# Shibodd/volume_path_tracer

Measured on AMD Instinct MI355X. Metric: Msamples/s (whole node) + achieved HBM GB/s, wdas_cloud 1920×1080, higher is better.
Workload: dtype f32

## Files before the change

### __graft_entry__.py

```python
from __future__ import annotations

import subprocess
import sys
from pathlib import Path

ROOT = Path(__file__).resolve().parent


def build() -> None:
    sys.path.insert(0, str(ROOT))
    from volume_path_tracer_amd import build as B

    B.build(verbose=True)
    subprocess.run(["make", "-s", "-C", str(ROOT / "oracle")], check=True)
    subprocess.run(["make", "-s", "-C", str(ROOT / "tests" / "native")], check=True)
    subprocess.run([sys.executable, "-B", "-c", "import sys; sys.path[:0] = [%r, %r]; import alpha_lib, denoise_lib; "
                    "alpha_lib.build_lib(); denoise_lib.build_lib()" % (str(ROOT), str(ROOT / "tests"))], check=True)
    import volume_path_tracer_amd
    from volume_path_tracer_amd import capi

    capi.lib()


def smoke() -> None:
    sys.path.insert(0, str(ROOT))
    sys.path.insert(0, str(ROOT / "tests"))
    import numpy as np
    import torch

    import oracle_lib as O
    from volume_path_tracer_amd.render import Integrator
    from volume_path_tracer_amd.scenes import SynthGrid, workload

    assert torch.cuda.is_available(), "smoke() needs a HIP device"
    wl = workload("c4", width=32, height=24, spp=2, grid_n=64)
    dens, temp = SynthGrid(1, 64).grid(), SynthGrid(2, 64).grid()
    it = Integrator(wl.cfg, dens, temp, device=0)
    jobs = wl.cfg.jobs_per_wave() * 2
    rec = torch.full((jobs * 64, 3), float("nan"), device="cuda:0")
    it.render_jobs(0, jobs, records=rec)
# ... 15 lines not shown
```

### include/vpt_gpu.h

```cpp
#ifndef VPT_GPU_H
#define VPT_GPU_H

#include <stddef.h>
#include <stdint.h>

#ifdef __cplusplus
extern "C" {
#endif

#define VPT_ABI_VERSION 1

enum {
  VPT_OK = 0,
  VPT_E_INVALID = 1,
  VPT_E_HIP = 2,
  VPT_E_IO = 3,
  VPT_E_PARSE = 4,
  VPT_E_NOMEM = 5,
  VPT_E_STATE = 6
};


typedef struct vpt_camera_params {
  float position[3];
// ... 98 lines not shown
int vpt_gpu_create(const vpt_configuration* cfg, const vpt_grid_desc* density,
                   const vpt_grid_desc* temperature, const float* blackbody_500x3, int device,
                   vpt_gpu_ctx** out);
int vpt_gpu_create_many(const vpt_configuration* cfg, const vpt_grid_desc* density,
                        const vpt_grid_desc* temperature, const float* blackbody_500x3, const int* devices, int n,
                        vpt_gpu_ctx** out);
typedef struct vpt_host_grids vpt_host_grids;
int vpt_grids_flatten(const vpt_grid_desc* density, const vpt_grid_desc* temperature, vpt_host_grids** out);
int vpt_gpu_create_from(const vpt_configuration* cfg, const vpt_host_grids* grids, const float* blackbody_500x3,
                        const int* devices, int n, vpt_gpu_ctx** out);
void vpt_grids_free(vpt_host_grids* grids);
int vpt_gpu_destroy(vpt_gpu_ctx* ctx);

int vpt_gpu_job_space(const vpt_gpu_ctx* ctx, uint64_t* jobs_per_wave, uint64_t* total_jobs);

int vpt_gpu_render_jobs(vpt_gpu_ctx* ctx, uint64_t jid_begin, uint64_t jid_count,
                        float* film_device, void* hip_stream);

enum { VPT_FILM_ATOMIC = 0, VPT_FILM_ORDERED = 1 };
int vpt_gpu_set_film_order(vpt_gpu_ctx* ctx, int mode, uint64_t max_bytes);
int vpt_gpu_film_order_info(const vpt_gpu_ctx* ctx, int* mode, uint64_t* buffer_bytes, uint64_t* ordered_launches,
                            uint64_t* atomic_launches);

int vpt_gpu_render_tiles(vpt_gpu_ctx* ctx, uint32_t tile_lo, uint32_t tile_hi, uint64_t wave_begin,
                         uint64_t wave_count, float* film_device, void* hip_stream);

int vpt_gpu_set_film_moments(vpt_gpu_ctx* ctx, float* m2_device);

int vpt_gpu_render_tile_list(vpt_gpu_ctx* ctx, const uint32_t* tiles, uint32_t n, uint64_t wave_begin,
                             uint64_t wave_count, float* film_device, void* hip_stream);

int vpt_gpu_tile_errors(vpt_gpu_ctx* ctx, const float* film_device, const float* m2_device, float abs_floor,
                        float* err_T_host, void* hip_stream);

typedef struct vpt_adaptive_params {
  float target_error, abs_floor;
  uint32_t min_waves, step_waves, max_waves;
} vpt_adaptive_params;

typedef struct vpt_adaptive_result {
  uint32_t rounds, tiles_at_max;
  uint64_t jobs_rendered, jobs_uniform;
  float max_error;
} vpt_adaptive_result;

int vpt_gpu_render_adaptive(vpt_gpu_ctx* ctx, const vpt_adaptive_params* p, float* film_device, float* m2_device,
// ... 138 lines not shown
```

### volume_path_tracer_amd/capi.py

```python
from __future__ import annotations

import ctypes as C
import os
from pathlib import Path

import numpy as np

PKG_DIR = Path(__file__).resolve().parent
LIB_DIR = PKG_DIR / "lib"
LIB_PATH = Path(os.environ["VPT_LIB"]) if os.environ.get("VPT_LIB") else LIB_DIR / "libvpt_amd.so"

VPT_OK = 0
VPT_BLACKBODY_ROWS = 500


class CameraParams(C.Structure):
    _fields_ = [("position", C.c_float * 3), ("look", C.c_float * 3), ("up", C.c_float * 3),
                ("vfov_deg", C.c_float), ("imaging_ratio", C.c_float)]


class WorkerParams(C.Structure):
    _fields_ = [("single_pixel_enabled", C.c_int32), ("use_jitter", C.c_int32),
                ("single_pixel_coord", C.c_int64 * 2),
                ("infinite_light_xyz", C.c_float * 3), ("infinite_light_multiplier", C.c_float),
# ... 75 lines not shown
    def make(cls, iterations=4, n_guides=0, sigma_l=4.0, rel_floor=1e-3, guide_sigma=None):
        if guide_sigma is None:
            guide_sigma = 0.2
        if np.isscalar(guide_sigma):
            guide_sigma = [guide_sigma] * n_guides
        gs = [float(v) for v in guide_sigma][:4]
        if len(gs) < min(n_guides, 4):
            raise ValueError("denoise: one guide_sigma per guide")
        gs += [1.0] * (4 - len(gs))
        return cls(int(iterations), int(n_guides), float(sigma_l), float(rel_floor), (C.c_float * 4)(*gs))


assert C.sizeof(DenoiseParams) == 32

EVENT_DTYPE = np.dtype([("jid", "<u8"), ("pixel", "<u4"), ("seq", "<u4"), ("type", "<u4"), ("v", "<f4", (7,))])
assert EVENT_DTYPE.itemsize == 48
DDA_ROW_DTYPE = np.dtype([("ijk", "<i4", (3,)), ("t", "<f4"), ("value", "<f4"), ("dim_getdim", "<u4"),
                          ("dim_nodeinfo", "<u4"), ("active", "<i4"), ("maximum", "<f4")])
assert DDA_ROW_DTYPE.itemsize == 36
VPT_RNG_REFERENCE, VPT_RNG_PIXEL = 0, 1
VPT_ORDER_JID, VPT_ORDER_COST_WAVE_MAJOR, VPT_ORDER_COST_TILE_MAJOR, VPT_ORDER_COST_TAIL = 0, 1, 2, 3
VPT_ORDER_COST_SAME_TILE = 4
VPT_FILM_ATOMIC, VPT_FILM_ORDERED = 0, 1
VPT_GATES_CONTEXT, VPT_GATES_LATENCY, VPT_GATES_FULL = 0, 1, 2
EVENT_NAMES = ("new_ray", "sampled_point", "null", "scatter_terminated", "scatter", "absorbed")


def _ptr(arr, ctype):
    if arr is None:
        return C.cast(None, C.POINTER(ctype))
    return arr.ctypes.data_as(C.POINTER(ctype))


class Grid:

    def __init__(self, *, map_mat, map_inv_mat, map_vec, background, bbox_min, bbox_max,
                 leaf_origin, leaf_values, leaf_max, leaf_value_mask=None,
                 tile_origin=None, tile_level=None, tile_value=None, tile_active=None,
                 lower_origin=None, upper_origin=None):
        self.leaf_origin = np.ascontiguousarray(leaf_origin, dtype=np.int32).reshape(-1, 3)
        n = self.leaf_origin.shape[0]
        self.leaf_values = np.ascontiguousarray(leaf_values, dtype=np.float32).reshape(n, 512)
        self.leaf_max = np.ascontiguousarray(leaf_max, dtype=np.float32).reshape(n)
        if leaf_value_mask is None:
            leaf_value_mask = np.full((n, 8), np.uint64(0xFFFFFFFFFFFFFFFF), dtype=np.uint64)
        self.leaf_value_mask = np.ascontiguousarray(leaf_value_mask, dtype=np.uint64).reshape(n, 8)
# ... 130 lines not shown
    if hasattr(L, "vpt_gpu_gate_info"):
        L.vpt_gpu_gate_info.argtypes = [vp, C.c_int, C.POINTER(C.c_int), C.POINTER(C.c_int)]
    L.vpt_gpu_launch_info.argtypes = [vp, C.POINTER(C.c_int), C.POINTER(C.c_int)]
    L.vpt_last_error.restype = C.c_char_p
    L.vpt_synth_grid.argtypes = [C.c_int, C.c_int]
    L.vpt_synth_grid.restype = gridp
    L.vpt_synth_free.argtypes = [gridp]
    L.vpt_grid_from_nanovdb.argtypes = [C.c_void_p, C.c_size_t, C.POINTER(gridp)]
    L.vpt_grid_read_nvdb.argtypes = [C.c_char_p, C.c_char_p, C.POINTER(gridp)]
    L.vpt_grid_free.argtypes = [gridp]
    L.vpt_film_to_srgb8.argtypes = [fp, C.c_int64, C.c_int64, C.POINTER(C.c_uint8)]
    L.vpt_gpu_trace_jobs.argtypes = [vp, C.c_uint64, C.c_uint64, vp, vp, C.c_uint64, C.POINTER(C.c_uint64), vp]
    L.vpt_gpu_majorant_trace.argtypes = [vp, fp, fp, fp, C.c_int, C.POINTER(C.c_int)]
    L.vpt_dda_trace.argtypes = [C.POINTER(GridDesc), fp, fp, vp, C.c_int, C.POINTER(C.c_int)]
    L.vpt_gpu_set_rng_mode.argtypes = [vp, C.c_int]
    if hasattr(L, "vpt_gpu_set_pixel_chunk"):
        L.vpt_gpu_set_pixel_chunk.argtypes = [vp, C.c_int]
    L.vpt_gpu_set_run_skipping.argtypes = [vp, C.c_int]
    L.vpt_gpu_kernel_variant.argtypes = [vp, C.POINTER(C.c_int), C.POINTER(C.c_int)]
    if hasattr(L, "vpt_gpu_set_film_order"):
        L.vpt_gpu_set_film_order.argtypes = [vp, C.c_int, C.c_uint64]
        L.vpt_gpu_film_order_info.argtypes = [vp, C.POINTER(C.c_int), C.POINTER(C.c_uint64),
                                              C.POINTER(C.c_uint64), C.POINTER(C.c_uint64)]
    L.vpt_gpu_set_job_order.argtypes = [vp, C.c_int]
    L.vpt_gpu_set_job_order_tail.argtypes = [vp, C.c_int]
    L.vpt_gpu_tile_costs.argtypes = [vp, fp, C.POINTER(C.c_uint32)]
    L.vpt_gpu_set_tile_costs.argtypes = [vp, fp]
    L.vpt_gpu_set_job_permutation.argtypes = [vp, C.POINTER(C.c_uint32), C.c_uint64]
    if hasattr(L, "vpt_gpu_set_latency_kernel"):
        L.vpt_gpu_set_latency_kernel.argtypes = [vp, C.c_int, C.c_int]
    if hasattr(L, "vpt_gpu_set_compaction"):
        L.vpt_gpu_set_compaction.argtypes = [vp, C.c_int]
        L.vpt_gpu_latency_kernel_info.argtypes = [vp, C.POINTER(C.c_int), C.POINTER(C.c_int)]
    if hasattr(L, "vpt_gpu_bind_thread_near"):
        L.vpt_gpu_bind_thread_near.argtypes = [vp, C.POINTER(C.c_int)]
    if hasattr(L, "vpt_gpu_stream_create"):
        L.vpt_gpu_stream_create.argtypes = [vp, C.POINTER(vp)]
        L.vpt_gpu_stream_destroy.argtypes = [vp, vp]
        L.vpt_gpu_stream_sync.argtypes = [vp, vp]
        L.vpt_gpu_film_alloc.argtypes = [vp, C.POINTER(vp)]
        L.vpt_gpu_film_free.argtypes = [vp, vp]
        L.vpt_gpu_film_flush_to_host.argtypes = [vp, vp, fp]
    if hasattr(L, "vpt_gpu_feed_open"):
        L.vpt_gpu_feed_open.argtypes = [vp, vp, vp, C.c_uint64, C.POINTER(vp)]
        L.vpt_gpu_feed_push.argtypes = [vp, C.POINTER(C.c_uint64), C.c_uint64]
        L.vpt_gpu_feed_close.argtypes = [vp]
# ... 45 lines not shown
```

### volume_path_tracer_amd/csrc/vpt_ctx.h

```cpp
#pragma once

#include <hip/hip_runtime.h>

#include <atomic>
#include <chrono>
#include <cstdint>
#include <mutex>
#include <string>
#include <vector>

#include "vpt_internal.h"
#include "vpt_launch.h"

#define VPT_HIP(call)                                                                                 \
  do {                                                                                                \
    hipError_t e_ = (call);                                                                           \
    if (e_ != hipSuccess)                                                                             \
      return ::vpt::set_error(VPT_E_HIP, std::string(#call " failed: ") + hipGetErrorString(e_));            \
  } while (0)

#ifndef VPT_DEFAULT_JOB_ORDER
#define VPT_DEFAULT_JOB_ORDER VPT_ORDER_COST_SAME_TILE
#endif

#ifndef VPT_DEFAULT_FULL_GATE_IDLE
#define VPT_DEFAULT_FULL_GATE_IDLE 4
#endif

#ifndef VPT_RUNS_MIN_FRACTION
#define VPT_RUNS_MIN_FRACTION 0.25
#endif

namespace vpt {
struct DeviceGrid {
  void* cells8 = nullptr;
  void* runs8 = nullptr;
  void* walk8 = nullptr;
  double run_fraction = 0.0;
  void* cells128 = nullptr;
  void* root = nullptr;
  void* bricks = nullptr;
  DevGrid dev{};
  size_t bytes = 0;
};

}

namespace vpt {
struct FeedLaunch {
  const uint64_t* word;
  uint64_t* ring;
  uint64_t mask;
  unsigned* error;
  uint64_t* started;
  uint64_t* waiting;
  uint32_t* tile_done;
};
struct BandLaunch {
  uint32_t tile_lo, tiles, waves, group;
  bool list = false;
};
}

struct vpt_gpu_feed;

struct vpt_gpu_ctx {
// ... 48 lines not shown
  hipEvent_t samples_done = nullptr;
  bool samples_used = false;
  uint64_t ordered_launches = 0, atomic_launches = 0;
  uint32_t* band_rank = nullptr;
  uint32_t band_rank_lo = 0, band_rank_hi = 0;
  uint32_t* list_dev = nullptr;
  uint32_t* list_slot_dev = nullptr;
  std::vector<uint32_t> list_host, list_slot_host;
  bool list_ranked = false;
  float* m2 = nullptr;
  float* tile_err = nullptr;
  float* gang_scratch = nullptr;
  uint64_t gang_scratch_bytes = 0;
  uint32_t* gang_waves = nullptr;
  void* denoise_scratch = nullptr;
  uint64_t denoise_scratch_bytes = 0;
  hipEvent_t denoise_done = nullptr;
  bool denoise_used = false;
  std::mutex denoise_mu;
  uint64_t frame_waves = 0, frame_jid_lo = 0;
  uint32_t frame_tile_lo = 0, frame_tiles = 0;
  float* frame_film = nullptr;
  double setup_ms[5] = {};
};

struct vpt_gpu_feed {
  vpt_gpu_ctx* ctx = nullptr;
  hipStream_t stream = nullptr;
  float* film = nullptr;
  uint64_t* block = nullptr;
  uint64_t* word = nullptr;
  uint32_t* error = nullptr;
  uint64_t* started = nullptr;
  uint64_t* waiting = nullptr;
  uint64_t* ring = nullptr;
  uint32_t* counts = nullptr;
  bool stage = false;
  uint32_t* done_dev = nullptr;
  float* pin_film = nullptr;
  uint32_t* pin_done = nullptr;
  std::vector<float> shown;
  std::vector<uint32_t> shown_done;
  hipStream_t copy_stream = nullptr;
  hipStream_t own_stream = nullptr;
  bool ring_clean = false;
  uint64_t cap = 0;
// ... 22 lines not shown
```

### volume_path_tracer_amd/csrc/vpt_gpu.hip

```cpp
#include <hip/hip_runtime.h>
#include <pthread.h>
#include <sched.h>
#include <unistd.h>

#include <algorithm>
#include <cmath>
#include <cstdio>
#include <cstdlib>
#include <cstring>
#include <fstream>
#include <functional>
#include <memory>
#include <atomic>
#include <mutex>
#include <chrono>
#include <string>
#include <thread>
#include <vector>

#include "vpt_ctx.h"
#include "vpt_kernels.h"
#include "vpt_denoise.h"

namespace vpt {
// ... 25 lines not shown
  int rc;
  const size_t need = h.cells8.size() * sizeof(int2) + h.runs8.size() + h.walk8.size() * sizeof(uint32_t) +
                      h.cells128.size() * sizeof(int2) + h.root.size() * sizeof(RootTileDev) +
                      h.bricks.size() * sizeof(float);
  size_t free_b = 0, total_b = 0;
  VPT_HIP(hipMemGetInfo(&free_b, &total_b));
  if (need > free_b)
    return set_error(VPT_E_NOMEM, "grid upload: needs " + std::to_string(need >> 20) + " MiB (" +
                                      std::to_string(h.dev.leaf_count) + " leaves x 9 KiB stencil pool + tables), " +
                                      std::to_string(free_b >> 20) + " MiB free on the device");
  if ((rc = upload(h.cells8.data(), h.cells8.size() * sizeof(int2), &d.cells8, d.bytes))) return rc;
  if ((rc = upload(h.runs8.data(), h.runs8.size(), &d.runs8, d.bytes))) return rc;
  if ((rc = upload(h.walk8.data(), h.walk8.size() * sizeof(uint32_t), &d.walk8, d.bytes))) return rc;
  d.run_fraction = h.run_fraction;
  if ((rc = upload(h.cells128.data(), h.cells128.size() * sizeof(int2), &d.cells128, d.bytes))) return rc;
  if ((rc = upload(h.root.data(), h.root.size() * sizeof(RootTileDev), &d.root, d.bytes))) return rc;
  if ((rc = upload(h.bricks.data(), h.bricks.size() * sizeof(float), &d.bricks, d.bytes))) return rc;
  d.dev.cells8 = (const int2*)d.cells8;
  d.dev.runs8 = (const uint8_t*)d.runs8;
  d.dev.walk8 = (const uint32_t*)d.walk8;
  d.dev.cells128 = (const int2*)d.cells128;
  d.dev.root = (const RootTileDev*)d.root;
  d.dev.bricks = (const float*)d.bricks;
  return VPT_OK;
}

static void free_grid(DeviceGrid& d) {
  (void)hipFree(d.cells8);
  (void)hipFree(d.runs8);
  (void)hipFree(d.walk8);
  (void)hipFree(d.cells128);
  (void)hipFree(d.root);
  (void)hipFree(d.bricks);
  d = DeviceGrid{};
}

}

namespace {

constexpr int kProfWords = 2 * vpt::PB_COUNT + vpt::PT_COUNT;
constexpr uint32_t kLaunchSlots = 64;
constexpr uint64_t kSpreadLanes = 6;

int wait_ctx(vpt_gpu_ctx* ctx);

int push_scene(vpt_gpu_ctx* ctx) {
  int rc = wait_ctx(ctx);
  if (rc) return rc;
  vpt::DevScene lat = ctx->scene;
  lat.gate_min = ctx->lat_gate[0];
  lat.gate_idle = ctx->lat_gate[1];
  lat.gate_eval = ctx->lat_gate[2];
  lat.gate_walk = ctx->lat_gate[3];
  lat.wave_lanes = ctx->lat_wave_lanes;
  VPT_HIP(hipMemcpyAsync(ctx->scene_dev, &ctx->scene, sizeof(vpt::DevScene), hipMemcpyHostToDevice, ctx->stream));
  VPT_HIP(hipMemcpyAsync(ctx->scene_lat_dev, &lat, sizeof(vpt::DevScene), hipMemcpyHostToDevice, ctx->stream));
// ... 133 lines not shown
  if (ctx->samples) {
    (void)hipFree(ctx->samples);
    ctx->samples = nullptr;
    ctx->samples_bytes = 0;
  }
  const hipError_t e = hipMalloc((void**)&ctx->samples, bytes);
  if (e != hipSuccess) {
    ctx->samples = nullptr;
    (void)hipGetLastError();
    return vpt::set_error(VPT_E_NOMEM, "ordered film: " + std::to_string(bytes >> 20) + " MiB sample buffer: " +
                                           hipGetErrorString(e) + " (vpt_gpu_set_film_order's max_bytes splits launches)");
  }
  ctx->samples_bytes = bytes;
  out = ctx->samples;
  return VPT_OK;
}

uint64_t ordered_cap(vpt_gpu_ctx* ctx, uint64_t want) {
  if (ctx->film_order_max) return ctx->film_order_max;
  if (want <= ctx->samples_bytes) return ctx->samples_bytes;
  size_t free_b = 0, total_b = 0;
  if (hipMemGetInfo(&free_b, &total_b) != hipSuccess) return ctx->samples_bytes;
  return (uint64_t)(free_b + ctx->samples_bytes) / 4 * 3;
}

}

int vpt::host::ctx_device(vpt_gpu_ctx* ctx) {
  hipError_t e = hipSetDevice(ctx->device);
  if (e != hipSuccess) return vpt::set_error(VPT_E_HIP, std::string("hipSetDevice: ") + hipGetErrorString(e));
  return VPT_OK;
}

int vpt::host::launch_tile_counts(vpt_gpu_ctx* ctx, float* film, const uint32_t* counts_dev, hipStream_t s) {
  const uint64_t npix = (uint64_t)ctx->scene.W * (uint64_t)ctx->scene.H;
  hipLaunchKernelGGL(vpt::vpt_tile_count_kernel, dim3((unsigned)((npix + 255) / 256)), dim3(256), 0, s, ctx->scene_dev,
                     film, counts_dev);
  VPT_HIP(hipGetLastError());
  return VPT_OK;
}

int vpt::host::render(vpt_gpu_ctx* ctx, uint64_t jid_begin, uint64_t jid_count, float* film, float* records,
                      void* stream_ptr, vpt_event* events, uint64_t event_cap, uint32_t* slot_out,
                      const vpt::FeedLaunch* feed, const vpt::BandLaunch* band) {
  if (!ctx) return vpt::set_error(VPT_E_INVALID, "render: null context");
  int rc = ctx_device(ctx);
// ... 332 lines not shown
  ctx->device = device;
  ctx->cfg = *cfg;
  ctx->setup_ms[0] = grids.flatten_ms;
  using clk = std::chrono::steady_clock;
  auto t = clk::now();
  auto lap = [&](int i) {
    const auto now = clk::now();
    ctx->setup_ms[i] += std::chrono::duration<double, std::milli>(now - t).count();
    t = now;
  };
  int rc = ctx_device(ctx.get());
  if (rc) return rc;
  lap(4);
  if ((rc = vpt::build_scene(*cfg, ctx->scene))) return rc;
  if ((rc = vpt::upload_grid(grids.density, ctx->density))) return rc;
  if (grids.has_temperature && (rc = vpt::upload_grid(grids.temperature, ctx->temperature))) return rc;
  lap(1);
  const bool has_temperature = grids.has_temperature;
  ctx->use_runs = !has_temperature && ctx->density.run_fraction >= VPT_RUNS_MIN_FRACTION;
  ctx->scene.density = ctx->density.dev;
  vpt::scene_finalize(ctx->scene);
  ctx->scene.temperature = ctx->temperature.dev;
  ctx->scene.has_temperature = has_temperature ? 1 : 0;
  ctx->scene.bb_lds_ok = has_temperature ? vpt::blackbody_rows_suffice(grids.temp_range, cfg->volume_parameters.temperature_scale,
                                                                    cfg->volume_parameters.temperature_offset, vpt::kBbLdsRows)
                                     : 0;

  std::vector<float> bb(501 * 3, 0.0f);
  if (blackbody_500x3)
    std::memcpy(bb.data(), blackbody_500x3, 500 * 3 * sizeof(float));
  else
    vpt::blackbody_table(bb.data());
  size_t scratch = 0;
  if ((rc = vpt::upload(bb.data(), bb.size() * sizeof(float), (void**)&ctx->bb, scratch))) return rc;
  if ((rc = vpt::upload(vpt::cie_table(), 471 * 3 * sizeof(float), (void**)&ctx->cie, scratch))) return rc;
  ctx->scene.bb = ctx->bb;
  ctx->scene.cie = ctx->cie;

  ctx->film_count = (uint64_t)cfg->output_size[0] * (uint64_t)cfg->output_size[1] * 4;
  VPT_HIP(hipMalloc((void**)&ctx->film, ctx->film_count * sizeof(float)));
  VPT_HIP(hipMemset(ctx->film, 0, ctx->film_count * sizeof(float)));
  VPT_HIP(hipMalloc((void**)&ctx->job_counter, kLaunchSlots * 2 * sizeof(unsigned long long)));
  for (uint32_t i = 0; i < kLaunchSlots; ++i)
    VPT_HIP(hipEventCreateWithFlags(&ctx->slot_done[i], hipEventDisableTiming));
  VPT_HIP(hipMalloc((void**)&ctx->counters, vpt::kCounterCount * sizeof(unsigned long long)));
  VPT_HIP(hipMemset(ctx->counters, 0, vpt::kCounterCount * sizeof(unsigned long long)));
// ... 594 lines not shown

int vpt_gpu_set_pixel_chunk(vpt_gpu_ctx* ctx, int chunk) {
  if (!ctx || chunk < 0 || (chunk & (chunk - 1)) != 0 || (chunk > 0 && ctx->scene.tile_area % (uint32_t)chunk != 0))
    return vpt::set_error(VPT_E_INVALID, "vpt_gpu_set_pixel_chunk: 0 or a power of two dividing the tile area");
  ctx->pixel_chunk = chunk;
  return VPT_OK;
}

int vpt_gpu_set_run_skipping(vpt_gpu_ctx* ctx, int mode) {
  if (!ctx || mode < -1 || mode > 1) return vpt::set_error(VPT_E_INVALID, "vpt_gpu_set_run_skipping: bad argument");
  if (mode == 1 && ctx->scene.has_temperature)
    return vpt::set_error(VPT_E_INVALID, "vpt_gpu_set_run_skipping: no run-skipping variant with a temperature grid");
  ctx->use_runs = mode < 0 ? (!ctx->scene.has_temperature && ctx->density.run_fraction >= VPT_RUNS_MIN_FRACTION) : mode == 1;
  return VPT_OK;
}

int vpt_gpu_kernel_variant(const vpt_gpu_ctx* ctx, int* has_temperature, int* run_skipping) {
  if (!ctx) return vpt::set_error(VPT_E_INVALID, "null context");
  if (has_temperature) *has_temperature = ctx->scene.has_temperature ? 1 : 0;
  if (run_skipping) *run_skipping = ctx->use_runs ? 1 : 0;
  return VPT_OK;
}

int vpt_gpu_set_film_order(vpt_gpu_ctx* ctx, int mode, uint64_t max_bytes) {
  if (!ctx || (mode != VPT_FILM_ATOMIC && mode != VPT_FILM_ORDERED))
    return vpt::set_error(VPT_E_INVALID, "vpt_gpu_set_film_order: bad argument");
  int rc = ctx_device(ctx);
  if (rc) return rc;
  ctx->film_order = mode;
  ctx->film_order_max = max_bytes;
  if (mode == VPT_FILM_ATOMIC && ctx->samples && ctx->open_feeds.load() == 0) {
    if (ctx->samples_used) VPT_HIP(hipEventSynchronize(ctx->samples_done));
    (void)hipFree(ctx->samples);
    ctx->samples = nullptr;
    ctx->samples_bytes = 0;
  }
  return VPT_OK;
}

int vpt_gpu_film_order_info(const vpt_gpu_ctx* ctx, int* mode, uint64_t* buffer_bytes, uint64_t* ordered_launches,
                            uint64_t* atomic_launches) {
  if (!ctx) return vpt::set_error(VPT_E_INVALID, "null context");
  if (mode) *mode = ctx->film_order;
  if (buffer_bytes) *buffer_bytes = ctx->samples_bytes;
  if (ordered_launches) *ordered_launches = ctx->ordered_launches;
  if (atomic_launches) *atomic_launches = ctx->atomic_launches;
// ... 403 lines not shown
```

### volume_path_tracer_amd/csrc/vpt_integrator.h

```cpp
#pragma once

#include <hip/hip_runtime.h>
#include <stdint.h>

#include "vpt_math.h"

namespace vpt {

struct RootTileDev {
  int32_t origin[3];
  float value;
  int32_t active;
  int32_t pad[3];
};

struct DevGrid {
  float mat[9], inv_mat[9], vec[3];
  float background;
  int32_t bbox_min[3], bbox_max[3];
  int32_t r8_org[3], r8_n[3];
  int32_t w8_org[3], w8_n[3];
  uint32_t w8_max;
  int32_t r128_org[3], r128_n[3];
  int32_t root_count, leaf_count;
  const int2* cells8;
  const uint8_t* runs8;
  const uint32_t* walk8;
  const int2* cells128;
  const RootTileDev* root;
  const float* bricks;
};

constexpr int kBrickVox = 576 * 4;
__host__ __device__ __forceinline__ int64_t brick_index(int32_t code, int32_t i, int32_t j, int32_t k) {
  return ((int64_t)code * 576 + ((j & 7) * 8 + (k & 7)) * 9 + (i & 7)) * 4;
}

struct Cell {
  int32_t code;
  float value;
};

__host__ __device__ __forceinline__ int32_t local_const(int32_t c) {
#if defined(__HIP_DEVICE_COMPILE__)
  int32_t r;
  asm volatile("v_mov_b32 %0, %1" : "=v"(r) : "i"(c));
  return r;
#else
  return c;
#endif
}
__host__ __device__ __forceinline__ float local_const(float c) {
#if defined(__HIP_DEVICE_COMPILE__)
  return __builtin_bit_cast(float, local_const(__builtin_bit_cast(int32_t, c)));
#else
  return c;
#endif
}
// ... 84 lines not shown
    v[1] = lo.y;
    v[2] = lo.z;
    v[3] = lo.w;
    v[4] = hi.x;
    v[5] = hi.y;
    v[6] = hi.z;
    v[7] = hi.w;
  } else {
#pragma unroll 1
    for (int q = 0; q < 8; ++q) {
      const float val = value_at(g, i + (q >> 2), j + ((q >> 1) & 1), k + (q & 1));
      v[0] = q == 0 ? val : v[0];
      v[1] = q == 1 ? val : v[1];
      v[2] = q == 2 ? val : v[2];
      v[3] = q == 3 ? val : v[3];
      v[4] = q == 4 ? val : v[4];
      v[5] = q == 5 ? val : v[5];
      v[6] = q == 6 ? val : v[6];
      v[7] = q == 7 ? val : v[7];
    }
  }
}

__host__ __device__ __forceinline__ float lerpf(float a, float b, float w) { return a + w * (b - a); }
__host__ __device__ __forceinline__ bool trilinear(const DevGrid& g, StencilCell& last, float x, float y, float z,
                                                   float& out) {
  float fi = floorf(x), fj = floorf(y), fk = floorf(z);
  float u = x - fi, v = y - fj, w = z - fk;
  int32_t i = (int32_t)fi, j = (int32_t)fj, k = (int32_t)fk;
  bool refresh = i != last.i || j != last.j || k != last.k;
  const int32_t dx = (i ^ last.i) | (j ^ last.j) | (k ^ last.k);
  const bool same_leaf = last.code >= 0 && dx >= 0 && dx < 8;
  Cell c;
  if (same_leaf) {
    c.code = last.code;
    c.value = 0.0f;
  } else {
    c = cell_at(g, i, j, k);
  }
  last.i = i;
  last.j = j;
  last.k = k;
  last.code = c.code;
  float s[8];
  fetch_stencil(g, c, i, j, k, s);
  out = lerpf(lerpf(lerpf(s[0], s[1], w), lerpf(s[2], s[3], w), v), lerpf(lerpf(s[4], s[5], w), lerpf(s[6], s[7], w), v), u);
  return refresh;
}
constexpr int32_t kNoCell = (int32_t)0x80000000;

__host__ __device__ __forceinline__ void map_inv(const DevGrid& g, float x, float y, float z, float& ox, float& oy, float& oz) {
  const float* m = g.inv_mat;
  float a = x - g.vec[0], b = y - g.vec[1], c = z - g.vec[2];
// ... 551 lines not shown
  if (u < 0.0f) {
    u = rng_uniform(ln.rng);
    if (Debug) env.tally(CNT_RNG_DRAWS, 1);
  }
  float total = ((0.0f + p_n) + p_a) + p_s;
  float uu = u * total;
  int ev;
  uu -= p_n;
  if (uu <= 0) {
    ev = 0;
  } else {
    uu -= p_a;
    ev = (uu <= 0) ? 1 : 2;
  }
  if (ev == 1) {
    if (Debug) env.event(ln, VPT_EV_ABSORBED, nullptr, nullptr, 0.0f);
    ln.state = ST_FINISH_T;
  } else if (ev == 2) {
    if (lc.depth++ >= S.max_depth) {
      if (Debug) env.event(ln, VPT_EV_SCATTER_TERMINATED, nullptr, nullptr, 0.0f);
      ln.state = ST_FINISH_T;
    } else {
      if (Debug) env.tally(CNT_SCATTERS, 1);
      for (int i = 0; i < 3; ++i) lc.ro[i] = cp[i];
      if (S.li_zero) {
        lc.Tr = -1.0f;
        ln.state = ST_NEE_DONE;
      } else {
        lc.Tr = local_const(1.0f);
        ln.shadow = 1;
        ln.state = ST_SHADOW;
      }
    }
  }
  if (Debug && ev == 0) env.event(ln, VPT_EV_NULL, nullptr, nullptr, 0.0f);
  if (ev != 0) ln.sm = SM_NONE;
}

template <bool HasTemp, bool Debug, class Env>
__host__ __device__ __forceinline__ void eval_collision(ScenePtr sp, const DevScene& S, const DevGrid& G, Lane& ln, Env& env) {
  LaneCold& lc = env.cold();
  const float sigma_maj = ln.s_dmaj * S.sigma_t;
  {
    const float dt_m = -math::logf_glibc_unit(lc.y_draw, env.logf_table()) / sigma_maj;
    const float tc = ln.s_t0 + math::div_by_recip(dt_m, ln.scale, ln.rscale);
    if (!(tc < ln.s_t1)) {
// ... 480 lines not shown
```

### volume_path_tracer_amd/csrc/vpt_kernels.h

```cpp
#pragma once

#include <hip/hip_runtime.h>

#include "vpt_alpha.h"
#include "vpt_internal.h"
#include "vpt_launch.h"

namespace vpt {

constexpr int kCounterCount = CNT_COUNT;
#ifndef VPT_WAVES_FAST
#define VPT_WAVES_FAST 7
#endif
#ifndef VPT_WAVES_SLOW
#define VPT_WAVES_SLOW 4
#endif
#ifndef VPT_WAVES_TEMP
#define VPT_WAVES_TEMP 6
#endif
#ifndef VPT_WAVES_LAT
#define VPT_WAVES_LAT 4
#endif

__shared__ LaneCold g_lane_cold[kBlockThreads];
// ... 984 lines not shown
    for (int i = 0; i < 3; ++i) dv[i] = S.cam_t[i] + (S.cam_L[i * 3] * rx + S.cam_L[i * 3 + 1] * ry);
    const float n = sqrtf(dv[0] * dv[0] + dv[1] * dv[1] + dv[2] * dv[2]);
    if (!(n > 0.0f)) continue;
    for (int i = 0; i < 3; ++i) dv[i] /= n;
    Lane ln;
    lane_init(ln);
    if (!begin_ray(G, ln, S.cam_pos, ray_dir_setup(G, dv))) continue;
    int steps = 0;
    float tau = 0.0f;
    while (ln.s_t1 < ln.T1 && steps < (1 << 16)) {
      begin_segment(ln);
      bool done;
      do {
        ++steps;
        done = hdda_step(G, ln);
      } while (!done && steps < (1 << 16));
      tau += S.sigma_t * ln.s_dmaj * (ln.s_t1 - ln.s_t0) * ln.scale;
    }
    c += (float)steps + 4.0f * tau;
  }
  cost[tile] = c;
}

__global__ __launch_bounds__(64) void vpt_alpha_kernel(const DevScene* scene, const uint32_t* rank, uint32_t sub,
                                                       float* alpha, float* tau) {
  const DevScene& S = *scene;
  const uint32_t area = S.tile_area, chunks = (area + 63u) / 64u;
  const uint32_t tb = blockIdx.x / chunks, q = (blockIdx.x - tb * chunks) * 64u + threadIdx.x;
  if ((uint64_t)tb >= S.T) return;
  const uint32_t t = rank[tb];
  const int32_t x0 = (int32_t)(t % (uint32_t)S.ntx) * S.tw, y0 = (int32_t)(t / (uint32_t)S.ntx) * S.th;
  const int32_t rw = min(S.W - x0, S.tw), rh = min(S.H - y0, S.th);
  if (q >= area || (int32_t)q >= rw * rh) return;
  const int32_t yl = (int32_t)q / rw, px = x0 + ((int32_t)q - yl * rw), py = y0 + yl;
  if (S.single_pixel_enabled && (px != S.sp_x || py != S.sp_y)) return;
  float a, od;
  alpha_pixel(S, px, py, sub, a, od);
  const uint64_t p = (uint64_t)py * (uint64_t)S.W + (uint64_t)px;
  alpha[p] = a;
  if (tau) tau[p] = od;
}

}
```

### volume_path_tracer_amd/render.py

```python
from __future__ import annotations

import ctypes as C
import threading
import time
from typing import Optional

import numpy as np

from . import capi


def ceildiv(a: int, b: int) -> int:
    return a // b + (a % b != 0)


class TileProvider:

    def __init__(self, img_size, waves: int, tile_size):
        self.img_w, self.img_h = int(img_size[0]), int(img_size[1])
        self.tile_w, self.tile_h = int(tile_size[0]), int(tile_size[1])
        self.ntx, self.nty = ceildiv(self.img_w, self.tile_w), ceildiv(self.img_h, self.tile_h)
        self.num_tiles = self.ntx * self.nty
        self.requested_waves = int(waves)
        self.max_wave_idx = 0
# ... 273 lines not shown

    def set_compaction(self, every: int) -> None:
        capi.check(capi.lib().vpt_gpu_set_compaction(self.h, int(every)), "vpt_gpu_set_compaction")

    def latency_kernel_info(self) -> dict:
        m, b = C.c_int(), C.c_int()
        capi.check(capi.lib().vpt_gpu_latency_kernel_info(self.h, C.byref(m), C.byref(b)), "vpt_gpu_latency_kernel_info")
        return {"mode": int(m.value), "resident_blocks_per_cu": int(b.value)}

    def kernel_variant(self) -> dict:
        t, r = C.c_int(), C.c_int()
        capi.check(capi.lib().vpt_gpu_kernel_variant(self.h, C.byref(t), C.byref(r)), "vpt_gpu_kernel_variant")
        return {"has_temperature": bool(t.value), "run_skipping": bool(r.value)}

    def set_film_order(self, mode: int, max_bytes: int = 0) -> None:
        capi.check(capi.lib().vpt_gpu_set_film_order(self.h, int(mode), int(max_bytes)), "vpt_gpu_set_film_order")

    def film_order_info(self) -> dict:
        m, b, o, a = C.c_int(), C.c_uint64(), C.c_uint64(), C.c_uint64()
        capi.check(capi.lib().vpt_gpu_film_order_info(self.h, C.byref(m), C.byref(b), C.byref(o), C.byref(a)),
                   "vpt_gpu_film_order_info")
        return {"mode": int(m.value), "buffer_bytes": int(b.value), "ordered_launches": int(o.value),
                "atomic_launches": int(a.value)}

    def set_job_order(self, mode: int) -> None:
        capi.check(capi.lib().vpt_gpu_set_job_order(self.h, int(mode)), "vpt_gpu_set_job_order")

    def set_job_order_tail(self, waves: int) -> None:
        capi.check(capi.lib().vpt_gpu_set_job_order_tail(self.h, int(waves)), "vpt_gpu_set_job_order_tail")

    def tile_costs(self):
        T = self.cfg.jobs_per_wave()
        cost, rank = np.zeros(T, np.float32), np.zeros(T, np.uint32)
        capi.check(capi.lib().vpt_gpu_tile_costs(self.h, cost.ctypes.data_as(C.POINTER(C.c_float)),
                                                  rank.ctypes.data_as(C.POINTER(C.c_uint32))), "vpt_gpu_tile_costs")
        return cost, rank

    def set_tile_costs(self, cost) -> None:
        c = np.ascontiguousarray(cost, np.float32)
        assert c.shape == (self.cfg.jobs_per_wave(),)
        capi.check(capi.lib().vpt_gpu_set_tile_costs(self.h, c.ctypes.data_as(C.POINTER(C.c_float))),
                   "vpt_gpu_set_tile_costs")

    def set_job_permutation(self, perm) -> None:
        p = np.ascontiguousarray(perm if perm is not None else [], np.uint32)
        capi.check(capi.lib().vpt_gpu_set_job_permutation(self.h, p.ctypes.data_as(C.POINTER(C.c_uint32)), p.size),
# ... 172 lines not shown
```

Baseline: 1675.

## Add dense stencil brick pool to bypass sparse cell lookup in trilinear sampling

Adds an optional dense pool holding a full 8^3 stencil brick for every cell of the level-8 grid, filled at setup by an expand kernel that copies the sparse bricks and synthesises the stencils for empty cells. Trilinear lookups inside the dense bounds then read two float4 directly from this pool and skip the cell/leaf indirection. An AUTO policy turns it on when the pool fits within one eighth of device memory. This trades extra memory and a one-time expansion pass for fewer dependent loads per sample. It also re-maps the scatter position through the density transform when temperature is present.

After: 1714 (median of 6 runs). 1.02x the previous value.

```diff
diff --git a/__graft_entry__.py b/__graft_entry__.py
--- a/__graft_entry__.py
+++ b/__graft_entry__.py
@@ -14,8 +14,9 @@
     B.build(verbose=True)
     subprocess.run(["make", "-s", "-C", str(ROOT / "oracle")], check=True)
     subprocess.run(["make", "-s", "-C", str(ROOT / "tests" / "native")], check=True)
-    subprocess.run([sys.executable, "-B", "-c", "import sys; sys.path[:0] = [%r, %r]; import alpha_lib, denoise_lib; "
-                    "alpha_lib.build_lib(); denoise_lib.build_lib()" % (str(ROOT), str(ROOT / "tests"))], check=True)
+    subprocess.run([sys.executable, "-B", "-c", "import sys; sys.path[:0] = [%r, %r]; import alpha_lib, denoise_lib, "
+                    "dense_pool_lib; alpha_lib.build_lib(); denoise_lib.build_lib(); dense_pool_lib.build_program()"
+                    % (str(ROOT), str(ROOT / "tests"))], check=True)
     import volume_path_tracer_amd
     from volume_path_tracer_amd import capi
 
diff --git a/include/vpt_gpu.h b/include/vpt_gpu.h
--- a/include/vpt_gpu.h
+++ b/include/vpt_gpu.h
@@ -144,6 +144,13 @@
 int vpt_gpu_film_order_info(const vpt_gpu_ctx* ctx, int* mode, uint64_t* buffer_bytes, uint64_t* ordered_launches,
                             uint64_t* atomic_launches);
 
+enum { VPT_POOL_SPARSE = 0, VPT_POOL_DENSE = 1, VPT_POOL_AUTO = 2 };
+int vpt_gpu_set_pool_layout(vpt_gpu_ctx* ctx, int layout);
+int vpt_gpu_set_pool_cap(vpt_gpu_ctx* ctx, uint64_t max_bytes);
+int vpt_gpu_pool_info(const vpt_gpu_ctx* ctx, int* layout, int* policy, uint64_t* sparse_bytes, uint64_t* dense_bytes,
+                      double* expand_ms);
+int vpt_gpu_debug_read_pool(vpt_gpu_ctx* ctx, int grid, uint64_t cell_begin, uint64_t cell_count, float* out);
+
 int vpt_gpu_render_tiles(vpt_gpu_ctx* ctx, uint32_t tile_lo, uint32_t tile_hi, uint64_t wave_begin,
                          uint64_t wave_count, float* film_device, void* hip_stream);
 
diff --git a/volume_path_tracer_amd/capi.py b/volume_path_tracer_amd/capi.py
--- a/volume_path_tracer_amd/capi.py
+++ b/volume_path_tracer_amd/capi.py
@@ -121,6 +121,7 @@
 VPT_ORDER_JID, VPT_ORDER_COST_WAVE_MAJOR, VPT_ORDER_COST_TILE_MAJOR, VPT_ORDER_COST_TAIL = 0, 1, 2, 3
 VPT_ORDER_COST_SAME_TILE = 4
 VPT_FILM_ATOMIC, VPT_FILM_ORDERED = 0, 1
+VPT_POOL_SPARSE, VPT_POOL_DENSE, VPT_POOL_AUTO = 0, 1, 2
 VPT_GATES_CONTEXT, VPT_GATES_LATENCY, VPT_GATES_FULL = 0, 1, 2
 EVENT_NAMES = ("new_ray", "sampled_point", "null", "scatter_terminated", "scatter", "absorbed")
 
@@ -297,6 +298,12 @@
         L.vpt_gpu_set_film_order.argtypes = [vp, C.c_int, C.c_uint64]
         L.vpt_gpu_film_order_info.argtypes = [vp, C.POINTER(C.c_int), C.POINTER(C.c_uint64),
                                               C.POINTER(C.c_uint64), C.POINTER(C.c_uint64)]
+    if hasattr(L, "vpt_gpu_set_pool_layout"):
+        L.vpt_gpu_set_pool_layout.argtypes = [vp, C.c_int]
+        L.vpt_gpu_set_pool_cap.argtypes = [vp, C.c_uint64]
+        L.vpt_gpu_pool_info.argtypes = [vp, C.POINTER(C.c_int), C.POINTER(C.c_int), C.POINTER(C.c_uint64),
+                                        C.POINTER(C.c_uint64), C.POINTER(C.c_double)]
+        L.vpt_gpu_debug_read_pool.argtypes = [vp, C.c_int, C.c_uint64, C.c_uint64, fp]
     L.vpt_gpu_set_job_order.argtypes = [vp, C.c_int]
     L.vpt_gpu_set_job_order_tail.argtypes = [vp, C.c_int]
     L.vpt_gpu_tile_costs.argtypes = [vp, fp, C.POINTER(C.c_uint32)]
diff --git a/volume_path_tracer_amd/csrc/vpt_ctx.h b/volume_path_tracer_amd/csrc/vpt_ctx.h
--- a/volume_path_tracer_amd/csrc/vpt_ctx.h
+++ b/volume_path_tracer_amd/csrc/vpt_ctx.h
@@ -40,8 +40,10 @@
   void* cells128 = nullptr;
   void* root = nullptr;
   void* bricks = nullptr;
+  void* dense = nullptr;
   DevGrid dev{};
   size_t bytes = 0;
+  size_t brick_bytes = 0, dense_bytes = 0;
 };
 
 }
@@ -136,6 +138,9 @@
   uint32_t frame_tile_lo = 0, frame_tiles = 0;
   float* frame_film = nullptr;
   double setup_ms[5] = {};
+  int pool_policy = VPT_POOL_AUTO;
+  uint64_t pool_cap = 0;
+  float pool_expand_ms = 0.0f;
 };
 
 struct vpt_gpu_feed {
diff --git a/volume_path_tracer_amd/csrc/vpt_gpu.hip b/volume_path_tracer_amd/csrc/vpt_gpu.hip
--- a/volume_path_tracer_amd/csrc/vpt_gpu.hip
+++ b/volume_path_tracer_amd/csrc/vpt_gpu.hip
@@ -71,6 +71,8 @@
   d.dev.cells128 = (const int2*)d.cells128;
   d.dev.root = (const RootTileDev*)d.root;
   d.dev.bricks = (const float*)d.bricks;
+  d.dev.dense = nullptr;
+  d.brick_bytes = h.bricks.size() * sizeof(float);
   return VPT_OK;
 }
 
@@ -81,7 +83,39 @@
   (void)hipFree(d.cells128);
   (void)hipFree(d.root);
   (void)hipFree(d.bricks);
+  (void)hipFree(d.dense);
   d = DeviceGrid{};
+}
+
+static uint64_t dense_pool_bytes(const DeviceGrid& d) {
+  if (!d.cells8) return 0;
+  return (uint64_t)d.dev.r8_n[0] * (uint64_t)d.dev.r8_n[1] * (uint64_t)d.dev.r8_n[2] * kBrickVox * sizeof(float);
+}
+
+static void free_dense(DeviceGrid& d) {
+  (void)hipFree(d.dense);
+  d.dense = nullptr;
+  d.dense_bytes = 0;
+  d.dev.dense = nullptr;
+}
+
+static int expand_dense(DeviceGrid& d) {
+  const uint64_t bytes = dense_pool_bytes(d);
+  if (bytes == 0) return VPT_OK;
+  const hipError_t e = hipMalloc(&d.dense, bytes);
+  if (e != hipSuccess) {
+    d.dense = nullptr;
+    (void)hipGetLastError();
+    return set_error(VPT_E_NOMEM, "dense stencil pool: " + std::to_string(bytes >> 20) + " MiB: " + hipGetErrorString(e));
+  }
+  d.dense_bytes = bytes;
+  const uint64_t cells = bytes / (kBrickVox * sizeof(float));
+  DevGrid g = d.dev;
+  g.dense = nullptr;
+  hipLaunchKernelGGL(vpt_dense_expand_kernel, dim3((unsigned)std::min<uint64_t>(cells, 1u << 20)), dim3(256), 0, nullptr,
+                     g, (float*)d.dense, cells);
+  VPT_HIP(hipGetLastError());
+  return VPT_OK;
 }
 
 }
@@ -261,6 +295,58 @@
   size_t free_b = 0, total_b = 0;
   if (hipMemGetInfo(&free_b, &total_b) != hipSuccess) return ctx->samples_bytes;
   return (uint64_t)(free_b + ctx->samples_bytes) / 4 * 3;
+}
+
+int apply_pool_layout(vpt_gpu_ctx* ctx, int policy) {
+  vpt::DeviceGrid* grids[2] = {&ctx->density, ctx->temperature.cells8 || ctx->temperature.bricks ? &ctx->temperature : nullptr};
+  uint64_t need = 0;
+  for (vpt::DeviceGrid* d : grids)
+    if (d) need += vpt::dense_pool_bytes(*d);
+  bool dense = policy == VPT_POOL_DENSE && need > 0;
+  if (policy == VPT_POOL_AUTO && need > 0) {
+    uint64_t cap = ctx->pool_cap;
+    if (cap == 0) {
+      size_t free_b = 0, total_b = 0;
+      VPT_HIP(hipMemGetInfo(&free_b, &total_b));
+      cap = (uint64_t)total_b / 8;
+    }
+    dense = need <= cap;
+  }
+  const bool have = ctx->density.dense != nullptr;
+  int rc = VPT_OK;
+  if (dense && !have) {
+    hipEvent_t ev[2] = {nullptr, nullptr};
+    VPT_HIP(hipEventCreate(&ev[0]));
+    VPT_HIP(hipEventCreate(&ev[1]));
+    (void)hipEventRecord(ev[0], nullptr);
+    for (vpt::DeviceGrid* d : grids)
+      if (d && rc == VPT_OK) rc = vpt::expand_dense(*d);
+    (void)hipEventRecord(ev[1], nullptr);
+    const hipError_t e = hipEventSynchronize(ev[1]);
+    if (rc == VPT_OK && e != hipSuccess) rc = vpt::set_error(VPT_E_HIP, std::string("dense stencil pool: ") + hipGetErrorString(e));
+    if (rc == VPT_OK) (void)hipEventElapsedTime(&ctx->pool_expand_ms, ev[0], ev[1]);
+    (void)hipEventDestroy(ev[0]);
+    (void)hipEventDestroy(ev[1]);
+    if (rc != VPT_OK) {
+      dense = false;
+      if (rc == VPT_E_NOMEM && policy == VPT_POOL_AUTO) rc = VPT_OK;
+    }
+  }
+  for (vpt::DeviceGrid* d : grids) {
+    if (!d) continue;
+    if (!dense) vpt::free_dense(*d);
+    d->dev.dense = (const float*)d->dense;
+  }
+  ctx->scene.density.dense = ctx->density.dev.dense;
+  ctx->scene.temperature.dense = ctx->temperature.dev.dense;
+  return rc;
+}
+
+int default_pool_policy() {
+  const char* v = std::getenv("VPT_POOL_LAYOUT");
+  if (v && !std::strcmp(v, "sparse")) return VPT_POOL_SPARSE;
+  if (v && !std::strcmp(v, "dense")) return VPT_POOL_DENSE;
+  return VPT_POOL_AUTO;
 }
 
 }
@@ -639,6 +725,9 @@
   vpt::scene_finalize(ctx->scene);
   ctx->scene.temperature = ctx->temperature.dev;
   ctx->scene.has_temperature = has_temperature ? 1 : 0;
+  ctx->pool_policy = default_pool_policy();
+  if ((rc = apply_pool_layout(ctx.get(), ctx->pool_policy))) return rc;
+  lap(1);
   ctx->scene.bb_lds_ok = has_temperature ? vpt::blackbody_rows_suffice(grids.temp_range, cfg->volume_parameters.temperature_scale,
                                                                     cfg->volume_parameters.temperature_offset, vpt::kBbLdsRows)
                                      : 0;
@@ -1279,6 +1368,51 @@
   return VPT_OK;
 }
 
+int vpt_gpu_set_pool_layout(vpt_gpu_ctx* ctx, int layout) {
+  if (!ctx || layout < VPT_POOL_SPARSE || layout > VPT_POOL_AUTO)
+    return vpt::set_error(VPT_E_INVALID, "vpt_gpu_set_pool_layout: bad argument");
+  if (ctx->open_feeds.load() > 0) return vpt::set_error(VPT_E_STATE, "vpt_gpu_set_pool_layout: a feed of this context is open");
+  if (ctx->frame_waves) return vpt::set_error(VPT_E_STATE, "vpt_gpu_set_pool_layout: a frame is open");
+  int rc = ctx_device(ctx);
+  if (rc) return rc;
+  if ((rc = wait_ctx(ctx))) return rc;
+  VPT_HIP(hipDeviceSynchronize());
+  ctx->pool_policy = layout;
+  rc = apply_pool_layout(ctx, layout);
+  const int prc = push_scene(ctx);
+  return rc ? rc : prc;
+}
+
+int vpt_gpu_set_pool_cap(vpt_gpu_ctx* ctx, uint64_t max_bytes) {
+  if (!ctx) return vpt::set_error(VPT_E_INVALID, "vpt_gpu_set_pool_cap: null context");
+  ctx->pool_cap = max_bytes;
+  return VPT_OK;
+}
+
+int vpt_gpu_pool_info(const vpt_gpu_ctx* ctx, int* layout, int* policy, uint64_t* sparse_bytes, uint64_t* dense_bytes,
+                      double* expand_ms) {
+  if (!ctx) return vpt::set_error(VPT_E_INVALID, "null context");
+  if (layout) *layout = ctx->density.dense ? VPT_POOL_DENSE : VPT_POOL_SPARSE;
+  if (policy) *policy = ctx->pool_policy;
+  if (sparse_bytes) sparse_bytes[0] = ctx->density.brick_bytes, sparse_bytes[1] = ctx->temperature.brick_bytes;
+  if (dense_bytes) dense_bytes[0] = ctx->density.dense_bytes, dense_bytes[1] = ctx->temperature.dense_bytes;
+  if (expand_ms) *expand_ms = ctx->pool_expand_ms;
+  return VPT_OK;
+}
+
+int vpt_gpu_debug_read_pool(vpt_gpu_ctx* ctx, int grid, uint64_t cell_begin, uint64_t cell_count, float* out) {
+  if (!ctx || !out || grid < 0 || grid > 1) return vpt::set_error(VPT_E_INVALID, "vpt_gpu_debug_read_pool: bad argument");
+  const vpt::DeviceGrid& d = grid ? ctx->temperature : ctx->density;
+  if (!d.dense) return vpt::set_error(VPT_E_STATE, "vpt_gpu_debug_read_pool: the grid has no dense pool");
+  const uint64_t brick = vpt::kBrickVox * sizeof(float), cells = d.dense_bytes / brick;
+  if (cell_begin > cells || cell_count > cells - cell_begin)
+    return vpt::set_error(VPT_E_INVALID, "vpt_gpu_debug_read_pool: cells outside the table");
+  int rc = ctx_device(ctx);
+  if (rc) return rc;
+  if (cell_count) VPT_HIP(hipMemcpy(out, (const char*)d.dense + cell_begin * brick, cell_count * brick, hipMemcpyDeviceToHost));
+  return VPT_OK;
+}
+
 int vpt_gpu_set_film_order(vpt_gpu_ctx* ctx, int mode, uint64_t max_bytes) {
   if (!ctx || (mode != VPT_FILM_ATOMIC && mode != VPT_FILM_ORDERED))
     return vpt::set_error(VPT_E_INVALID, "vpt_gpu_set_film_order: bad argument");
diff --git a/volume_path_tracer_amd/csrc/vpt_integrator.h b/volume_path_tracer_amd/csrc/vpt_integrator.h
--- a/volume_path_tracer_amd/csrc/vpt_integrator.h
+++ b/volume_path_tracer_amd/csrc/vpt_integrator.h
@@ -29,11 +29,15 @@
   const int2* cells128;
   const RootTileDev* root;
   const float* bricks;
+  const float* dense;
 };
 
 constexpr int kBrickVox = 576 * 4;
 __host__ __device__ __forceinline__ int64_t brick_index(int32_t code, int32_t i, int32_t j, int32_t k) {
   return ((int64_t)code * 576 + ((j & 7) * 8 + (k & 7)) * 9 + (i & 7)) * 4;
+}
+__host__ __device__ __forceinline__ int64_t dense_index(uint32_t cell, int32_t i, int32_t j, int32_t k) {
+  return (int64_t)(((uint64_t)cell * 576u + (uint32_t)(((j & 7) * 8 + (k & 7)) * 9 + (i & 7))) * 4u);
 }
 
 struct Cell {
@@ -164,6 +168,16 @@
   }
 }
 
+__host__ __device__ __forceinline__ void dense_square(const DevGrid& g, int32_t a, int32_t b, int32_t c, int32_t s,
+                                                      float out[4]) {
+  const int32_t x = s % 9, yz = s / 9;
+  const int32_t i = g.r8_org[0] + a * 8 + x, j = g.r8_org[1] + b * 8 + (yz >> 3), k = g.r8_org[2] + c * 8 + (yz & 7);
+  out[0] = value_at(g, i, j, k);
+  out[1] = value_at(g, i, j, k + 1);
+  out[2] = value_at(g, i, j + 1, k);
+  out[3] = value_at(g, i, j + 1, k + 1);
+}
+
 __host__ __device__ __forceinline__ float lerpf(float a, float b, float w) { return a + w * (b - a); }
 __host__ __device__ __forceinline__ bool trilinear(const DevGrid& g, StencilCell& last, float x, float y, float z,
                                                    float& out) {
@@ -171,6 +185,19 @@
   float u = x - fi, v = y - fj, w = z - fk;
   int32_t i = (int32_t)fi, j = (int32_t)fj, k = (int32_t)fk;
   bool refresh = i != last.i || j != last.j || k != last.k;
+  if (g.dense) {
+    const int32_t a = (i - g.r8_org[0]) >> 3, b = (j - g.r8_org[1]) >> 3, c = (k - g.r8_org[2]) >> 3;
+    if ((uint32_t)a < (uint32_t)g.r8_n[0] && (uint32_t)b < (uint32_t)g.r8_n[1] && (uint32_t)c < (uint32_t)g.r8_n[2]) {
+      const float4* p = reinterpret_cast<const float4*>(g.dense + dense_index(mad_index(a, b, c, g.r8_n), i, j, k));
+      const float4 lo = p[0], hi = p[1];
+      last.i = i;
+      last.j = j;
+      last.k = k;
+      last.code = -1;
+      out = lerpf(lerpf(lerpf(lo.x, lo.y, w), lerpf(lo.z, lo.w, w), v), lerpf(lerpf(hi.x, hi.y, w), lerpf(hi.z, hi.w, w), v), u);
+      return refresh;
+    }
+  }
   const int32_t dx = (i ^ last.i) | (j ^ last.j) | (k ^ last.k);
   const bool same_leaf = last.code >= 0 && dx >= 0 && dx < 8;
   Cell c;
@@ -768,6 +795,11 @@
       ln.state = ST_FINISH_T;
     } else {
       if (Debug) env.tally(CNT_SCATTERS, 1);
+      if (HasTemp) {
+        const DevScene Sr = *opaque(sp);
+        const float t = local_value(ln.s_t0);
+        map_fwd(Sr.density, ln.e[0] + ln.d[0] * t, ln.e[1] + ln.d[1] * t, ln.e[2] + ln.d[2] * t, cp[0], cp[1], cp[2]);
+      }
       for (int i = 0; i < 3; ++i) lc.ro[i] = cp[i];
       if (S.li_zero) {
         lc.Tr = -1.0f;
diff --git a/volume_path_tracer_amd/csrc/vpt_kernels.h b/volume_path_tracer_amd/csrc/vpt_kernels.h
--- a/volume_path_tracer_amd/csrc/vpt_kernels.h
+++ b/volume_path_tracer_amd/csrc/vpt_kernels.h
@@ -1030,6 +1030,25 @@
   cost[tile] = c;
 }
 
+__global__ __launch_bounds__(256) void vpt_dense_expand_kernel(DevGrid g, float* dense, uint64_t cells) {
+  const uint64_t ny = (uint64_t)g.r8_n[1], nz = (uint64_t)g.r8_n[2];
+  for (uint64_t cell = blockIdx.x; cell < cells; cell += gridDim.x) {
+    const int32_t code = cell8_code(g.cells8[cell].x);
+    float4* dst = reinterpret_cast<float4*>(dense + cell * (uint64_t)kBrickVox);
+    if (code >= 0) {
+      const float4* src = reinterpret_cast<const float4*>(g.bricks + (int64_t)code * kBrickVox);
+      for (int32_t s = (int32_t)threadIdx.x; s < kBrickVox / 4; s += (int32_t)blockDim.x) dst[s] = src[s];
+    } else {
+      const int32_t c = (int32_t)(cell % nz), b = (int32_t)((cell / nz) % ny), a = (int32_t)(cell / (nz * ny));
+      for (int32_t s = (int32_t)threadIdx.x; s < kBrickVox / 4; s += (int32_t)blockDim.x) {
+        float v[4];
+        dense_square(g, a, b, c, s, v);
+        dst[s] = make_float4(v[0], v[1], v[2], v[3]);
+      }
+    }
+  }
+}
+
 __global__ __launch_bounds__(64) void vpt_alpha_kernel(const DevScene* scene, const uint32_t* rank, uint32_t sub,
                                                        float* alpha, float* tau) {
   const DevScene& S = *scene;
diff --git a/volume_path_tracer_amd/render.py b/volume_path_tracer_amd/render.py
--- a/volume_path_tracer_amd/render.py
+++ b/volume_path_tracer_amd/render.py
@@ -319,6 +319,24 @@
                    "vpt_gpu_film_order_info")
         return {"mode": int(m.value), "buffer_bytes": int(b.value), "ordered_launches": int(o.value),
                 "atomic_launches": int(a.value)}
+
+    def set_pool_layout(self, layout: int, cap_bytes: int | None = None) -> None:
+        if cap_bytes is not None:
+            capi.check(capi.lib().vpt_gpu_set_pool_cap(self.h, int(cap_bytes)), "vpt_gpu_set_pool_cap")
+        capi.check(capi.lib().vpt_gpu_set_pool_layout(self.h, int(layout)), "vpt_gpu_set_pool_layout")
+
+    def pool_info(self) -> dict:
+        la, po, ms = C.c_int(), C.c_int(), C.c_double()
+        sp, de = (C.c_uint64 * 2)(), (C.c_uint64 * 2)()
+        capi.check(capi.lib().vpt_gpu_pool_info(self.h, C.byref(la), C.byref(po), sp, de, C.byref(ms)), "vpt_gpu_pool_info")
+        return {"layout": int(la.value), "policy": int(po.value), "sparse_bytes": (int(sp[0]), int(sp[1])),
+                "dense_bytes": (int(de[0]), int(de[1])), "expand_ms": float(ms.value)}
+
+    def debug_read_pool(self, grid: int, cell_begin: int, cell_count: int) -> np.ndarray:
+        out = np.empty((int(cell_count), 2304), dtype=np.float32)
+        capi.check(capi.lib().vpt_gpu_debug_read_pool(self.h, int(grid), int(cell_begin), int(cell_count),
+                                                      out.ctypes.data_as(C.POINTER(C.c_float))), "vpt_gpu_debug_read_pool")
+        return out
 
     def set_job_order(self, mode: int) -> None:
         capi.check(capi.lib().vpt_gpu_set_job_order(self.h, int(mode)), "vpt_gpu_set_job_order")
```
